# ossamaAhmed/blackbox_mpc

Hardware: AMD Instinct MI355X
Metric: MPC control-steps/sec (agent-control-steps; Pendulum true model, CEM N=500 H=30) (higher is better)
Workload: dtype f32; 1 GPU; BASELINE cfg2: Pendulum-v0 true dynamics, CEM, num_agents=1/GPU, N=500, H=30, 5 iters, k=50, closed loop (the model is the environment); parallelism=single GPU

## Files before the change

### blackbox_mpc_amd/csrc/bbmpc.hip

```cpp
#include "engine.hpp"
#include "abi_util.hpp"
#include "engine_util.hpp"
#include "kernels_corr.hpp"
#include "kernels_elite_carry.hpp"

#include <math.h>
#include <stdio.h>
#include <stdlib.h>
#include <atomic>
#include <functional>
#include <chrono>
#include <mutex>
#include <set>
#include <thread>
#include <utility>

namespace bbmpc {

static std::mutex g_engines_mu;
static std::set<Engine*> g_engines;
static std::atomic<int> g_resident_handles{0};
void note_resident_handle() { g_resident_handles.fetch_add(1, std::memory_order_relaxed); }

void stop_foreign_residents(Engine* self) {
// ... 107 lines not shown
        const bool per_agent = (c.quirks & BBMPC_CMAES_PER_AGENT) != 0;
        const long nn = per_agent ? (long)H * U : (long)A * H * U;
        REQUIRE(nn <= 4096, BBMPC_E_UNSUPPORTED,
                "CMA-ES joint dimension num_agents*H*U > 4096: use BBMPC_CMAES_PER_AGENT (the reference's own "
                "[N,n,n] map_fn stack cannot run at this size either, cma_es.py:13)");
        REQUIRE(per_agent || c.num_agents_global <= c.num_agents, BBMPC_E_UNSUPPORTED,
                "coupled CMA-ES sums rewards over ALL agents and does not shard; use BBMPC_CMAES_PER_AGENT");
        REQUIRE(k <= 1024, BBMPC_E_UNSUPPORTED, "num_elite > 1024 not supported");
    }

    if (c.population_global != 0 || c.population_offset != 0) {
        REQUIRE(c.population_global >= N && c.population_offset >= 0 && c.population_offset + N <= c.population_global, BBMPC_E_INVALID,
                "population_offset / population_global: this handle's particles must lie inside the global population");
        if (c.population_global > N) {
            REQUIRE(c.optimizer != BBMPC_OPT_NONE, BBMPC_E_UNSUPPORTED, "population sharding needs an optimizer (evaluate-only handles roll out what they are given)");
            if (c.optimizer == BBMPC_OPT_CMAES)
                REQUIRE(k <= N && k <= 1024, BBMPC_E_UNSUPPORTED, "sharded CMA-ES: num_elite must not exceed this rank's share of the population (nor 1024)");
        }
    }
    int ndev = 0;
    if (hipGetDeviceCount(&ndev) != hipSuccess || ndev <= 0)
        throw HipError(BBMPC_E_NO_DEVICE, "no HIP device available: this library has no CPU fallback");
    if (c.device >= 0) {
        REQUIRE(c.device < ndev, BBMPC_E_NO_DEVICE, "bbmpc_config.device out of range");
        HIP_CHECK(hipSetDevice(c.device));
    }
    HIP_CHECK(hipGetDevice(&device));
    HIP_CHECK(hipDeviceGetAttribute(&cu_count, hipDeviceAttributeMultiprocessorCount, device));
    {
        int least = 0, greatest = 0;
        HIP_CHECK(hipDeviceGetStreamPriorityRange(&least, &greatest));
        if (!(own_stream = masked_stream_from_env("BBMPC_STREAM_CUS", cu_count)))
            HIP_CHECK(hipStreamCreateWithPriority(&own_stream, hipStreamNonBlocking, greatest));
    }
    stream = own_stream;
    init_tnq_table();

    if (const char* fm = getenv("BBMPC_FUSED")) fused_mode = atoi(fm);
    {
        auto flag = [](const char* n) { return getenv(n) != nullptr; };
        auto ival = [](const char* n, int dflt) { const char* v = getenv(n); return v ? atoi(v) : dflt; };
        sw.cma_svd_v1 = flag("BBMPC_CMA_SVD_V1"); sw.cma_svd_rounds = flag("BBMPC_CMA_SVD_ROUNDS");
        sw.cma_svd_general = flag("BBMPC_CMA_SVD_GENERAL");
        sw.cma_svd_gram = flag("BBMPC_CMA_SVD_GRAM");
        sw.cma_coop = flag("BBMPC_CMA_COOP"); sw.cma_nb = ival("BBMPC_CMA_NB", 0);
        sw.cma_eigh = ival("BBMPC_CMA_EIGH", 1); sw.cma_eigh_fail = flag("BBMPC_CMA_EIGH_FAIL");
        sw.cma_fused = flag("BBMPC_CMA_FUSED");
        sw.mlp_generic = flag("BBMPC_MLP_GENERIC");
        { const int b = ival("BBMPC_MLP_BF16", 0); sw.mlp_bf16 = (b == 1 || b == 3) ? b : 0; }
        sw.mlp_pair = ival("BBMPC_MLP_PAIR", -1); sw.mlp_q4 = ival("BBMPC_MLP_Q4", -1); sw.mlp_q4s = ival("BBMPC_MLP_Q4S", ival("BBMPC_MLP_Q4R", 1)); sw.mlp_w4 = ival("BBMPC_MLP_W4", 1); sw.pi2_skip_init = ival("BBMPC_PI2_SKIP_INIT", 1); sw.step_graph = ival("BBMPC_STEP_GRAPH", 1); sw.cma_small3 = ival("BBMPC_CMA_SMALL3", 1);
        sw.refit_wgs = ival("BBMPC_REFIT_WGS", 0);
        sw.mlp_wave = ival("BBMPC_MLP_WAVE", 1);
        sw.linger_us = std::max(0, ival("BBMPC_LINGER_US", 200));
        linger_test_quit = ival("BBMPC_LINGER_TEST_QUIT", 0) - 1;
        host_seq = (uint32_t)ival("BBMPC_TEST_HOST_SEQ", 0);
        sw.balance = ival("BBMPC_BALANCE", 0);
        sw.ilp = ival("BBMPC_ILP", 1) == 2 ? 2 : 1;
        sw.refit_v1 = flag("BBMPC_REFIT_V1");
        sw.zero_copy = !flag("BBMPC_NO_ZERO_COPY");
        sw.host_poll = !flag("BBMPC_NO_HOST_POLL");
        sw.mlp_no_half_tail = flag("BBMPC_MLP_NO_HALF_TAIL");
        sw.dbg = flag("BBMPC_DBG");
        sw.prof_reward_mlp = flag("BBMPC_PROF_REWARD_MLP");
        user_stepwise_only = flag("BBMPC_USER_STEPWISE");
        if (c.optimizer != BBMPC_OPT_NONE) {
            ps_loopback = auto_split > 1 ? auto_split : ival("BBMPC_POPSHARD_LOOPBACK", 0);
            ps_force = flag("BBMPC_POPSHARD_FORCE");
        }
    }
    HU = H * U;
    Nst = ((std::max(N, 1) + 63) / 64) * 64;
    rec = U + S + 1;
    lo.assign(c.action_low, c.action_low + U);
    hi.assign(c.action_high, c.action_high + U);
    upload(d_lo, lo);
    upload(d_hi, hi);
    d_state.alloc((size_t)A * S);
    d_record.alloc((size_t)A * rec);
    d_action.alloc((size_t)A * U);
    d_action.zero(stream);
    if (c.optimizer != BBMPC_OPT_NONE) {
        std::vector<float> m((size_t)A * HU), v((size_t)A * HU);
        for (int i = 0; i < A * HU; ++i) {
            const int u = i % U;
            m[i] = (lo[u] + hi[u]) / 2.0f;
            const float d = lo[u] - hi[u];
            v[i] = (d * d) / 16.0f;
        }
        upload(d_prev_mean, m);
        upload(d_var0, v);
        d_mean.alloc(m.size());
        d_var.alloc(m.size());
        d_sigma.alloc(m.size());
        d_samples.alloc((size_t)A * HU * Nst);
        d_rewards.alloc((size_t)A * Nst);
        d_penalty.alloc((size_t)A * Nst);
        d_elites.alloc((size_t)A * std::max(k, 1));
        const size_t big = (size_t)A * HU * Nst;
        if (c.optimizer == BBMPC_OPT_SPSA) {
            d_cand_a.alloc(big);
            d_cand_b.alloc(big);
            d_rewards2.alloc((size_t)A * Nst);
        }
        if (c.optimizer == BBMPC_OPT_CMAES) {
            d_cand_a.alloc(big);
            cma_init();
// ... 2145 lines not shown
```

### blackbox_mpc_amd/csrc/bbmpc_fused.hip

```cpp
#define BBMPC_TU_FUSED
#include "engine.hpp"
#include "engine_util.hpp"

#include <atomic>
#include <chrono>

namespace bbmpc {

void bbmpc_tu_fused_upload_tnq(const float2* table) { tnq_upload(table); }

bool Engine::use_fused() const {
    if (cfg.dynamics != BBMPC_DYN_PENDULUM || cfg.reward != BBMPC_REW_PENDULUM) return false;
    if (pop_sharded()) return false;
    if (particles_on()) return false;
    if (corr_on()) return false;
    if (carry_on()) return false;
    if (prior_on()) return false;
    if (grad_on()) return false;
    if (cfg.optimizer == BBMPC_OPT_SPSA) {
        if (iters > FUSED_MAX_SPSA_ITERS) return false;
    } else if (cfg.optimizer != BBMPC_OPT_RANDOM_SEARCH && cfg.optimizer != BBMPC_OPT_CEM && cfg.optimizer != BBMPC_OPT_PI2) {
        return false;
    }
    if (fused_mode == 0) return false;
    if (fused_mode == 1) return true;
    return (long)N <= 2048 || A >= 64;
}

static void note_inst(Engine& e, int opt, bool samples_lds, bool fastm, int inj, int ilp, bool linger) {
    snprintf(e.dominant_inst, sizeof(e.dominant_inst), "k_fused_pendulum<%d, %s, %s, %d, %d, %s>", opt, samples_lds ? "true" : "false",
             fastm ? "true" : "false", inj, ilp, linger ? "true" : "false");
}

template <int OPT, bool FASTM, int INJ, int ILP>
static void launch_fused4(Engine& e, FusedArgs& fa, int threads, size_t lds_base, size_t lds_samples) {
#ifdef BBMPC_KERNEL_DBG
    const size_t limit = 158 * 1024;
#else
    const size_t limit = 160 * 1024;
#endif
    if (lds_base + lds_samples <= limit) {
        fa.test_quit_agent = -1;
        if constexpr (INJ == 2 && FASTM && ILP == 1) {
            if (e.linger_launch && e.subset_n == 0 && fa.done_flag && e.tail.event == nullptr) {
                auto fl = k_fused_pendulum<OPT, true, FASTM, INJ, ILP, true>;
                note_inst(e, OPT, true, FASTM, INJ, ILP, true);
                ensure_max_lds((const void*)fl, (int)limit);
                if (e.rec != kCompletionRecordFloats) throw HipError(BBMPC_E_HIP, "internal: the resident pendulum kernel's record is not 5 floats");
                for (int a = 0; a < e.A; ++a) {
                    volatile uint32_t* m = e.mbox_host(a);
                    volatile uint32_t* cl = e.ack_host(a);
                    for (int i = 0; i < 16; ++i) cl[i] = (fa.done_value - 1u) & 0xffffu;                    for (int i = 0; i < 13; ++i) m[i] = fa.done_value & 0xffffu;
                    m[15] = fa.done_value;
                    *(volatile uint32_t*)e.gone_host(a) = 0u;
                }
                std::atomic_thread_fence(std::memory_order_release);
                fa.done_flag = e.sync_dev(e.ack_host(0));
                fa.mbox = e.sync_dev(e.mbox_host(0));
                fa.gone = e.sync_dev(e.gone_host(0));
                fa.linger_ticks = (unsigned)e.sw.linger_us * 100u;
                fa.test_quit_agent = e.linger_test_quit;
                hipLaunchKernelGGL(fl, dim3(e.A), dim3(threads), lds_base + lds_samples, e.stream, fa);
                HIP_CHECK(hipGetLastError());
                e.resident_alive = true;
                if (!e.mbox_pub.load(std::memory_order_relaxed)) {
                    e.mbox_pub_agents = e.A;
                    e.mbox_pub.store(e.mbox_host(0), std::memory_order_release);
                    note_resident_handle();
                }
                return;
            }
        }
        if (e.subset_n > 0) {
            auto fs = k_fused_pendulum<OPT, true, FASTM, INJ, ILP>;
            note_inst(e, OPT, true, FASTM, INJ, ILP, false);
            ensure_max_lds((const void*)fs, (int)limit);
            fa.amap = reinterpret_cast<const int*>(e.sync_dev(e.amap_host()));
            hipLaunchKernelGGL(fs, dim3(e.subset_n), dim3(threads), lds_base + lds_samples, e.stream, fa);
            HIP_CHECK(hipGetLastError());
            e.subset_n = 0;
            return;
        }
        auto fn = k_fused_pendulum<OPT, true, FASTM, INJ, ILP>;
        note_inst(e, OPT, true, FASTM, INJ, ILP, false);
        ensure_max_lds((const void*)fn, (int)limit);
        launch_with_tail(e, fn, dim3(e.A), dim3(threads), lds_base + lds_samples, fa);
    } else {
        auto fn = k_fused_pendulum<OPT, false, FASTM, INJ, ILP>;
        note_inst(e, OPT, false, FASTM, INJ, ILP, false);
        launch_with_tail(e, fn, dim3(e.A), dim3(threads), lds_base, fa);
    }
    HIP_CHECK(hipGetLastError());
}

template <int OPT>
static void launch_fused(Engine& e, FusedArgs& fa, int ilp, int threads, size_t lds_base, size_t lds_samples, int inj_layout) {
    const bool fastm = !e.fix(BBMPC_STRICT_MATH);
    const int inj = fa.inj == nullptr ? 0 : inj_layout;
#define LF(F, I)                                                                              \
    do {                                                                                      \
        if (ilp == 2) launch_fused4<OPT, F, I, 2>(e, fa, threads, lds_base, lds_samples);    \
        else launch_fused4<OPT, F, I, 1>(e, fa, threads, lds_base, lds_samples);             \
    } while (0)
    if (inj == 2) {
        if (fastm) launch_fused4<OPT, true, 2, 1>(e, fa, threads, lds_base, lds_samples);
        else launch_fused4<OPT, false, 2, 1>(e, fa, threads, lds_base, lds_samples);
    } else if (fastm && !inj) LF(true, 0);
    else if (fastm && inj) LF(true, 1);
    else if (!fastm && !inj) LF(false, 0);
    else LF(false, 1);
#undef LF
}

__global__ void k_noise_fill(RngKey key, uint32_t rstream, int kind , int n_it, int N, int Nst, int A, int Q,
                             int agent_offset, float4* __restrict__ out) {
    const int idx = blockIdx.x * blockDim.x + threadIdx.x;
    if (idx >= N * Q) return;
    const int n = idx / Q, q = idx % Q;
    const int z = blockIdx.y;
    const int a = z % A, it = (z / A) % n_it, s = z / (A * n_it);
    key.step += (uint32_t)s;
    const U4 w = rng_block(key, rstream, (uint32_t)it, (uint32_t)n, (uint32_t)(agent_offset + a), (uint32_t)(4 * q));
    float4 v;
    if (kind == 1) v = make_float4(word_to_uniform(w.x), word_to_uniform(w.y), word_to_uniform(w.z), word_to_uniform(w.w));
    else if (kind == 2) v = make_float4(word_to_rademacher(w.x), word_to_rademacher(w.y), word_to_rademacher(w.z), word_to_rademacher(w.w));
    else v = make_float4(word_to_trunc_normal(w.x), word_to_trunc_normal(w.y), word_to_trunc_normal(w.z), word_to_trunc_normal(w.w));
    out[(((size_t)s * n_it + it) * A + a) * Nst * Q + (size_t)n * Q + q] = v;
}

void Engine::launch_noise_fill(int64_t chunk, int buf, hipStream_t on) {
    const bool rs = cfg.optimizer == BBMPC_OPT_RANDOM_SEARCH, sp = cfg.optimizer == BBMPC_OPT_SPSA;
    const int n_it = rs ? 1 : iters, Q = (HU + 3) / 4;
    dim3 grid((N * Q + 255) / 256, A * n_it * pf_steps), block(256);
    hipLaunchKernelGGL(k_noise_fill, grid, block, 0, on, key((uint32_t)(chunk * pf_steps)), rs ? 2u : (sp ? 3u : 1u), rs ? 1 : (sp ? 2 : 0), n_it,
                       N, Nst, A, Q, cfg.agent_offset, reinterpret_cast<float4*>(d_noise_pf[buf].p));
    HIP_CHECK(hipGetLastError());
}

void Engine::optimize_fused(const float* d_state_in, int add_noise, float* d_record_out, float* d_next_out, uint32_t step) {
    FusedArgs fa;
    memset(&fa, 0, sizeof(fa));
    fa.N = N; fa.A = A; fa.H = H; fa.U = U; fa.HU = HU; fa.Nst = Nst; fa.k = k; fa.iters = iters;
    fa.agent_offset = cfg.agent_offset;
// ... 26 lines not shown
        ensure_trace();
        fa.t_rewards = t_rewards.p; fa.t_mean = t_mean.p; fa.t_var = t_var.p; fa.t_elites = t_elites.p; fa.t_passes = t_passes.p; fa.t_samples = t_samples.p;
        if (cfg.optimizer == BBMPC_OPT_SPSA) {
            if (!t_rewards2.p) t_rewards2.alloc((size_t)A * Nst * std::max(iters, 1));
            fa.t_rewards2 = t_rewards2.p;
        }
    }
#ifdef BBMPC_KERNEL_DBG
    static long long* dbg_buf = nullptr;
    if (sw.dbg) {
        if (!dbg_buf) {
            HIP_CHECK(hipHostMalloc((void**)&dbg_buf, 64 * 8, hipHostMallocDefault));
            memset(dbg_buf, 0, 64 * 8);
        }
        if (dbg_buf[42]) {
            const long long* d = dbg_buf;
            fprintf(stderr, "[dbg] last resident pass, 10ns units rel. to its start:");
            for (int i = 0; i <= 1 + iters * 4; ++i) fprintf(stderr, " %lld", d[i] - d[0]);
            fprintf(stderr, "\n[dbg] iter0 per-wave rollout end:");
            for (int i = 24; i < 32; ++i) fprintf(stderr, " %lld", d[i] - d[0]);
            fprintf(stderr, "\n[dbg] request accepted %lld  first model step %lld  completion stored %lld\n", d[42] - d[0], d[44] - d[0], d[43] - d[0]);
            const long long sel = d[iters > 0 ? 4 * iters : 0];
            fprintf(stderr, "[dbg] tail rel. to the last selection: tail start %lld  noise applied %lld  model step %lld  record stored %lld  published %lld  last barrier %lld  carry stored %lld\n",
                    d[38] - sel, d[35] - sel, d[36] - sel, d[37] - sel, d[43] - sel, d[1 + iters * 4] - sel, d[34] - sel);
            dbg_buf[42] = 0;
        }
        fa.dbg = dbg_buf;
    }
#endif
    fa.key = key(step);
    const int pf_nit = cfg.optimizer == BBMPC_OPT_RANDOM_SEARCH ? 1 : iters;
    if (pf_mode < 0) {
        const char* ev = getenv("BBMPC_NOISE_PREFETCH");
        pf_step_floats = U == 1 ? noise_step_floats(pf_nit, A, Nst, H) : (size_t)pf_nit * A * Nst * ((HU + 3) / 4) * 4;
        const size_t budget = (size_t)128 << 20;
        pf_steps = pf_step_floats ? (int)std::min<size_t>(8, budget / (pf_step_floats * 4)) : 0;
        pf_mode = ((ev ? atoi(ev) != 0 : true) && pf_steps >= 1 && U == 1) ? 1 : 0;
        if (pf_mode) {
            {
                int least = 0, greatest = 0;
                HIP_CHECK(hipDeviceGetStreamPriorityRange(&least, &greatest));
                HIP_CHECK(hipStreamCreateWithPriority(&pf_stream, hipStreamNonBlocking, greatest));
            }
            HIP_CHECK(hipEventCreateWithFlags(&pf_free, hipEventDisableTiming));
            for (int b = 0; b < 2; ++b) {
                const size_t pad = noise_pad_floats(H);
                d_noise_pf[b].alloc(noise_alloc_floats(pf_steps, pf_nit, A, Nst, H));
                HIP_CHECK(hipMemset(d_noise_pf[b].p + pf_step_floats * pf_steps, 0xff, pad * sizeof(float)));
                HIP_CHECK(hipEventCreateWithFlags(&pf_done[b], hipEventDisableTiming));
            }
        }
    }
    const bool use_pf = pf_mode == 1 && fa.inj == nullptr && pf_nit > 0;
    if (use_pf) {
        const int64_t c = (int64_t)step / pf_steps;
        const int pb = (int)(c & 1), nb = pb ^ 1;
        if (pf_chunk[pb] != c) {
            if (pf_inflight[pb]) HIP_CHECK(hipStreamWaitEvent(stream, pf_done[pb], 0));
            launch_noise_fill(c, pb, stream);
            pf_chunk[pb] = c; pf_waited[pb] = true; pf_inflight[pb] = false;
        } else if (!pf_waited[pb]) {
            HIP_CHECK(hipStreamWaitEvent(stream, pf_done[pb], 0));
            pf_waited[pb] = true; pf_inflight[pb] = false;
        }
        fa.inj = d_noise_pf[pb].p + (size_t)((int64_t)step - c * pf_steps) * pf_step_floats;
        fa.pf_buf[0] = d_noise_pf[0].p; fa.pf_buf[1] = d_noise_pf[1].p;
        fa.pf_step_floats = pf_step_floats; fa.pf_chunk_floats = pf_step_floats * (size_t)pf_steps;
        if (pf_chunk[nb] != c + 1) {
            HIP_CHECK(hipEventRecord(pf_free, stream));
            HIP_CHECK(hipStreamWaitEvent(pf_stream, pf_free, 0));
            launch_noise_fill(c + 1, nb, pf_stream);
            HIP_CHECK(hipEventRecord(pf_done[nb], pf_stream));
            pf_chunk[nb] = c + 1; pf_waited[nb] = false; pf_inflight[nb] = true;
        }
    }
    int ilp = 1;
    ilp = sw.ilp;
    if (use_pf) ilp = 1;
    const int per = (N + ilp - 1) / ilp;
    const int threads = std::min(1024, std::max(((per + 63) / 64) * 64, ((std::max(k, 1) + 63) / 64) * 64));
    const int HUp = (HU + 3) & ~3, kp = (std::max(k, 1) + 3) & ~3;
    static_assert(TOPK_HIST_WORDS % 4 == 0, "every piece of the carve is a multiple of 16 bytes");
    static_assert(TOPK_HIST_WORDS_NARROW % 4 == 0, "every piece of the carve is a multiple of 16 bytes");
    const int hist_words = cfg.optimizer == BBMPC_OPT_CEM ? TOPK_HIST_WORDS : TOPK_HIST_WORDS_NARROW;
    const size_t lds_base = (size_t)(Nst + 3 * HUp + kp + 64 + hist_words + 2 * kp) * 4;
    const size_t lds_samples = (size_t)HU * Nst * 4;
    prof_begin();
    switch (cfg.optimizer) {
        case BBMPC_OPT_RANDOM_SEARCH: launch_fused<FOPT_RS>(*this, fa, ilp, threads, lds_base, lds_samples, use_pf ? 2 : 1); break;
        case BBMPC_OPT_CEM: launch_fused<FOPT_CEM>(*this, fa, ilp, threads, lds_base, lds_samples, use_pf ? 2 : 1); break;
        case BBMPC_OPT_SPSA: {
            const bool fastm = !fix(BBMPC_STRICT_MATH);
            if (use_pf) {
                if (fastm) launch_fused4<FOPT_SPSA, true, 2, 1>(*this, fa, threads, lds_base, lds_samples);
                else launch_fused4<FOPT_SPSA, false, 2, 1>(*this, fa, threads, lds_base, lds_samples);
            } else if (fa.inj) {
                if (fastm) launch_fused4<FOPT_SPSA, true, 1, 1>(*this, fa, threads, lds_base, lds_samples);
                else launch_fused4<FOPT_SPSA, false, 1, 1>(*this, fa, threads, lds_base, lds_samples);
            } else {
                if (fastm) launch_fused4<FOPT_SPSA, true, 0, 1>(*this, fa, threads, lds_base, lds_samples);
                else launch_fused4<FOPT_SPSA, false, 0, 1>(*this, fa, threads, lds_base, lds_samples);
            }
            break;
        }
        default: launch_fused<FOPT_PI2>(*this, fa, ilp, threads, lds_base, lds_samples, use_pf ? 2 : 1); break;
    }
// ... 70 lines not shown
```

### blackbox_mpc_amd/csrc/engine.hpp

```cpp
#pragma once
#include <hip/hip_ext.h>
#include <hip/hip_runtime.h>
#include <stdint.h>
#include <string.h>

#include <algorithm>
#include <atomic>
#include <map>
#include <stdexcept>
#include <string>
#include <vector>

#include "../../include/bbmpc.h"
#include "comm.hpp"
#include "completion_line.hpp"
#include "kernels_cma.hpp"
#include "kernels_eigh.hpp"
#include "kernels_eigh_small.hpp"
#include "kernels_fused.hpp"
#include "kernels_fused_cma.hpp"
#include "kernels_fused_pso.hpp"
#include "kernels_mlp.hpp"
#include "kernels_mlp_xform.hpp"
#include "kernels_mlp_q4s.hpp"
// ... 93 lines not shown
        if (flag) attached = true;
        return {flag, count, value};
    }
};

struct Engine {
    bbmpc_config cfg;
    int N, A, H, U, S, HU, Nst, iters, k;
    int rec;
    std::vector<float> lo, hi;
    hipStream_t own_stream = nullptr, stream = nullptr;
    int cu_count = 0;
    int device = 0;
    uint32_t step_counter = 0;
    hipGraphExec_t step_graph = nullptr;
    uint64_t step_graph_sig = 0;
    uint64_t step_warm_sig = 0;
    int step_graph_warm = 0;
    uint32_t mutations = 0;
    uint32_t* step_words_dev = nullptr;
    uint32_t* step_words = nullptr;
    uint32_t step_mirror[2] = {0, 0};
    void ensure_step_words();
    bool step_capturing = false;
    int64_t calls_graph = 0;
    int64_t graph_capture_failures = 0;
    bool last_step_steady = false;
    void invalidate_step_graph() {
        ++mutations;
        step_graph_warm = 0;
        if (step_graph) { (void)hipGraphExecDestroy(step_graph); step_graph = nullptr; }
    }
    bool trace_on = false, profiling = false;
    int prof_every = 1;
    uint64_t prof_seq = 0;
    bool prof_this = false;
    int fused_mode = -1;
    struct Switches {
        bool cma_svd_v1 = false, cma_svd_rounds = false, cma_svd_general = false, cma_svd_gram = false, cma_fused = false, cma_coop = false;
        bool cma_eigh_fail = false;
        int cma_eigh = 1;
        int cma_nb = 0;
        bool mlp_generic = false;
        int mlp_bf16 = 0;
        int mlp_pair = -1, mlp_q4 = -1;
        int mlp_w4 = 1;
        int mlp_q4s = 1;
        int cma_small3 = 1;
        int step_graph = 1;
        int pi2_skip_init = 1;
        int refit_wgs = 0;
        int mlp_wave = 1;
        int linger_us = 200;
        int balance = 0;
        int ilp = 1;
        bool refit_v1 = false;
        bool zero_copy = true;
        bool mlp_no_half_tail = false;
        bool host_poll = true;
        bool prof_reward_mlp = false;
        bool dbg = false;
    } sw;

    DevBuf<float> d_lo, d_hi, d_state, d_record, d_action;
    DevBuf<float> d_prev_mean, d_var0, d_mean, d_var, d_sigma;
    DevBuf<float> d_samples, d_rewards, d_penalty;
    DevBuf<int> d_elites;
    bool mlp_ready = false;
    MlpDesc mlp;
    int mlp_nw = 1;
    DevBuf<float> d_wpack[MLP_MAX_LAYERS], d_wpack4[MLP_MAX_LAYERS], d_bpack[MLP_MAX_LAYERS], d_wraw[MLP_MAX_LAYERS], d_braw[MLP_MAX_LAYERS], d_wq4[MLP_MAX_LAYERS], d_wq4s0, d_w4pack, d_wbf[MLP_MAX_LAYERS], d_stats;
    DevBuf<float> d_fin_next, d_fin_rew, d_step_act;
    DevBuf<float> d_cand_a, d_cand_b, d_rewards2, d_vel, d_pbest, d_pbest_r, d_gbest, d_gbest_r, d_cond;
    DevBuf<int> d_gidx;
    DevBuf<float> t_rewards2;
    bool pso_seeded = false;
    int cma_G = 0, cma_n = 0;
    CmaConst cma_c;
    DevBuf<float> c_w, c_m, c_sigma, c_C, c_B, c_Dd, c_ps, c_pc, c_BD, c_z, c_Ye, c_xm, c_ym, c_evec, c_eval, c_E;
    DevBuf<int> c_eidx, c_info;
    DevBuf<unsigned> c_sync;
    DevBuf<float> e_d, e_e, e_tau, e_Vt, e_alpha, e_lam, e_Z, e_Z2, e_P, e_Tf;
    DevBuf<unsigned> e_flags;
    bool cma_use_eigh_small() const { return sw.cma_eigh && cma_n >= 2 && cma_n <= ES_N && !sw.cma_svd_v1 && !sw.cma_svd_rounds && !sw.cma_svd_general && !sw.cma_svd_gram; }
    bool cma_use_eigh() const { return sw.cma_eigh && cma_n > 128 && cma_n <= EIGH_MAX_N && (cma_n & 3) == 0 && !sw.cma_svd_v1 && !sw.cma_svd_rounds && !sw.cma_svd_general && !sw.cma_svd_gram; }
    void cma_eigh_launch(const CmaArgs& q);
    hipStream_t eigh_side = nullptr;
    hipEvent_t eigh_ev[2] = {nullptr, nullptr};
    int eigh_side_state = -1;
    DevBuf<float> d_eval_rew, d_step_c;
    DevBuf<float> d_stage;
    int stage_depth = 0;
    std::map<int, DevBuf<float>> inj;
    DevBuf<float> t_rewards, t_mean, t_var, t_samples;
    DevBuf<int> t_elites;
    DevBuf<int> t_passes;
    DevBuf<int> t_cma_stats;
    DevBuf<float> t_cma_B, t_cma_C, t_cma_D;
    float* h_pin = nullptr;
    float* h_pin_dev = nullptr;
    size_t h_pin_n = 0;
    DevBuf<float> d_noise_pf[2];
    RecordComm rc;
    DevBuf<float> d_record_slot[RecordComm::kSlots];
    float* h_record_stage[RecordComm::kSlots] = {nullptr, nullptr};
    bool gather_deferred[RecordComm::kSlots] = {false, false};
// ... 337 lines not shown
```

### blackbox_mpc_amd/csrc/kernels_fused.hpp

```cpp
#pragma once
#include <type_traits>

#include "kernels_opt.hpp"
#include "kernels_refit.hpp"
#include "kernels_rollout.hpp"
#include "noise_extent.hpp"
#include "topk.hpp"

namespace bbmpc {

constexpr int FOPT_RS = 1;
constexpr int FOPT_CEM = 2;
constexpr int FOPT_PI2 = 3;
constexpr int FOPT_SPSA = 4;
constexpr int FUSED_MAX_SPSA_ITERS = 16;

struct FusedArgs {
    int N, A, H, U, HU, Nst, k, iters;
    int agent_offset;
    int fix_q1, fix_q7, add_noise;
    int warm_start;
    unsigned* done_flag;
    unsigned* done_count;
    unsigned done_value;
// ... 8 lines not shown
    float* samples_g;
    const float* inj;
    const float* inj_expl;
    float* record;
    float* next_state;
    float spsa_ak[FUSED_MAX_SPSA_ITERS], spsa_ck[FUSED_MAX_SPSA_ITERS];
    float* t_rewards2;
    float* t_rewards;
    float* t_mean;
    float* t_var;
    int* t_elites;
    float* t_samples;
    long long* dbg;
    RngKey key;
    const unsigned* mbox;
    unsigned* gone;
    unsigned linger_ticks;
    int test_quit_agent;
    const int* amap;
    const float* pf_buf[2];
    unsigned long long pf_step_floats, pf_chunk_floats;
    int* t_passes;
};


#ifdef BBMPC_KERNEL_DBG
#define BB_DBG(slot) do { if (p.dbg && tid == 0 && a == 0) dbg_lds[(slot)] = (long long)wall_clock64(); } while (0)
#else
#define BB_DBG(slot) do {} while (0)
#endif

__device__ __forceinline__ float block_min(float v, float* red, int tid, int nw) {
    v = wave_min(v);
    if ((tid & 63) == 0) red[tid >> 6] = v;
    __syncthreads();
    float r = red[(tid & 63) < nw ? (tid & 63) : 0];
    r = wave_min(r);
    __syncthreads();
    return r;
}
__device__ __forceinline__ float block_sum(float v, float* red, int tid, int nw) {
    v = wave_sum(v);
    if ((tid & 63) == 0) red[tid >> 6] = v;
    __syncthreads();
    float r = ((tid & 63) < nw) ? red[tid & 63] : 0.0f;
    r = wave_sum(r);
    __syncthreads();
    return r;
}

#ifndef BBMPC_FUSED_ACTIONS_AHEAD
#define BBMPC_FUSED_ACTIONS_AHEAD 1
#endif
template <int OPT, bool SAMPLES_LDS, bool FASTM, int INJ, int ILP, bool LINGER = false>
__global__ void k_fused_pendulum(FusedArgs p) {
    extern __shared__ __attribute__((aligned(16))) float smem[];
    const int a = p.amap ? p.amap[blockIdx.x] : (int)blockIdx.x;
    const int tid = threadIdx.x;
    const int nthr = blockDim.x;
    const int nw = nthr >> 6;
    const int HUp = (p.HU + 3) & ~3;
    const int kp = (p.k + 3) & ~3;
    float* rew = smem;
    float* mean = rew + p.Nst;
    float* var = mean + HUp;
    float* sigma = var + HUp;
    int* eidx = (int*)(sigma + HUp);
    float* red = (float*)(eidx + kp);
    uint32_t* hist = (uint32_t*)(red + 64);
    unsigned long long* ekeys = (unsigned long long*)(hist + (OPT == FOPT_CEM ? TOPK_HIST_WORDS : TOPK_HIST_WORDS_NARROW));
    float* samp = SAMPLES_LDS ? (float*)(ekeys + kp) : (p.samples_g + (size_t)a * p.HU * p.Nst);
#ifdef BBMPC_KERNEL_DBG
    __shared__ long long dbg_lds[48];
#endif
    const PendulumModel model{p.fix_q1 != 0};
    const float lo = p.lo[0], hi = p.hi[0];
    RngKey key_s = p.key;
    const float* inj_s = p.inj;
    int add_noise_s = p.add_noise;
    unsigned done_value_s = p.done_value;
    if (tid < 3) red[60 + tid] = p.state[a * 3 + tid];
    const bool keep_init = LINGER && OPT != FOPT_RS && p.HU <= nthr;
    [[maybe_unused]] float m_keep = 0.0f, v_keep = 0.0f, s_keep = 0.0f;
    auto dist_init = [&](bool from_keep) {
        if (from_keep) {
            if (tid < p.HU) {
                mean[tid] = m_keep;
                var[tid] = v_keep;
                sigma[tid] = (OPT == FOPT_CEM && p.warm_start) ? cem_sigma(m_keep, v_keep, lo, hi) : s_keep;
            }
        } else {
            for (int j = tid; j < p.HU; j += nthr) {
                const float m = p.prev_mean[a * p.HU + j];
                const float v = p.var0[a * p.HU + j];
                const float sg = (OPT == FOPT_CEM) ? cem_sigma(m, v, lo, hi) : ((OPT == FOPT_SPSA) ? 0.0f : sqrtf(v));
                mean[j] = m;
                var[j] = v;
                sigma[j] = sg;
                if (keep_init) { m_keep = m; v_keep = v; s_keep = sg; }
            }
        }
    };
    typedef float pfvec4 __attribute__((ext_vector_type(4)));
    typedef const __attribute__((address_space(1))) pfvec4* pfvec4p;
    [[maybe_unused]] pfvec4 pf0 = {0.0f, 0.0f, 0.0f, 0.0f}, pf1 = {0.0f, 0.0f, 0.0f, 0.0f};
    [[maybe_unused]] auto prefetch_first = [&](const float* base, int it_n) {
        if constexpr (INJ == 2) {
            const int Q = (p.HU + 3) >> 2;
            if (tid < p.N) {
                const pfvec4p q = (pfvec4p)(reinterpret_cast<const float4*>(base) + noise_block_index(it_n, p.A, a, p.Nst, tid, Q));
                pf0 = q[0];
                if (OPT != FOPT_SPSA) pf1 = q[1];
            }
        }
    };
    dist_init(false);
    __syncthreads();
    float s0 = red[60], s1 = red[61], s2 = red[62];
    if (p.iters > 0) prefetch_first(inj_s, 0);
    auto noise_term = [&]() {
        FinalArgs fa;
        fa.A = p.A; fa.U = 1; fa.S = 3;
        fa.agent_offset = p.agent_offset;
        fa.fix_q1 = p.fix_q1; fa.fix_q7 = p.fix_q7;
        fa.add_noise = add_noise_s;
        fa.lo = p.lo; fa.hi = p.hi;
        fa.inj = p.inj_expl;
        fa.key = key_s;
        fa.key.q_per_agent = 1;
        return exploration_noise(fa, a, 0, lo, hi);
    };
    const bool tail_lanes = LINGER ? tid < 64 : tid == 0;
    auto tail = [&](float act_in) {
        BB_DBG(38);
        float s[3] = {s0, s1, s2};
        float act[1];
        act[0] = add_noise_s ? exploration_apply(act_in, noise_term(), lo, hi) : act_in;
        BB_DBG(35);
        const float r = model.step(s, act);
        BB_DBG(36);
        if constexpr (LINGER) {
            const unsigned tag = done_value_s & 0xffffu;
            const float f = tid < 2 ? act[0] : (tid < 4 ? s[0] : (tid < 6 ? s[1] : (tid < 8 ? s[2] : r)));
            const unsigned bits = __float_as_uint(f);
            unsigned w = ((tid & 1) ? (bits & 0xffff0000u) : (bits << 16)) | tag;
            if (tid >= 10) w = tag;
            if (tid == 15) w = done_value_s;
            if (tid < 16) __hip_atomic_store(p.done_flag + a * 16 + tid, w, __ATOMIC_RELAXED, __HIP_MEMORY_SCOPE_SYSTEM);
            BB_DBG(37);
        } else {
            float* rec = p.record + (size_t)a * 5;
            rec[0] = act[0];
            rec[1] = s[0];
            rec[2] = s[1];
            rec[3] = s[2];
            rec[4] = r;
            if (p.next_state) {
                p.next_state[a * 3 + 0] = s[0];
                p.next_state[a * 3 + 1] = s[1];
                p.next_state[a * 3 + 2] = s[2];
            }
            BB_DBG(37);
            publish_records_done(p.done_flag, p.done_count, done_value_s, gridDim.x);
        }
        BB_DBG(43);
    };
    for (;;) {

        float action0 = (OPT == FOPT_RS) ? 0.0f : mean[0];

        BB_DBG(0);
#ifdef BBMPC_KERNEL_DBG
        if (p.dbg && tid == 0 && a == 0) dbg_lds[40] = (long long)clock64();
#endif
        for (int it = 0; it < p.iters; ++it) {
            BB_DBG(1 + it * 4);
            const float* inj = (INJ == 1) ? inj_s + ((size_t)it * p.A + a) * p.HU * p.Nst : nullptr;
            const int nblk = p.H >> 2, rem = p.H & 3;
            const uint32_t rstream = (OPT == FOPT_RS) ? 2u : 1u;
            auto with_q1 = [&](auto&& body) {
                if constexpr (FASTM) {
                    if (p.fix_q1 != 0) { body(std::true_type{}); return; }
                }
                body(std::false_type{});
            };
            if constexpr (OPT == FOPT_SPSA) {
                const float ck = p.spsa_ck[it];
                const int nb4 = (p.H + 3) >> 2;
                with_q1([&](auto Q1c) {
                constexpr bool Q1 = decltype(Q1c)::value;
                for (int n = tid; n < p.N; n += nthr) {
                    Roller<FASTM> rp, rm;
                    rp.init(p.fix_q1 != 0, s0, s1, s2);
                    rm.init(p.fix_q1 != 0, s0, s1, s2);
                    float tp = 0.0f, tm = 0.0f, pp = 0.0f, pm = 0.0f;
                    typedef float gvec4s __attribute__((ext_vector_type(4)));
                    typedef const __attribute__((address_space(1))) gvec4s* gvec4sp;
                    [[maybe_unused]] gvec4sp mine4 = nullptr;
                    [[maybe_unused]] gvec4s cur4 = {1.0f, 1.0f, 1.0f, 1.0f};
                    if constexpr (INJ == 2) {
                        mine4 = (gvec4sp)(reinterpret_cast<const float4*>(inj_s) + noise_block_index(it, p.A, a, p.Nst, n, nb4));
                        if (n == tid) cur4 = pf0;
                        else cur4 = mine4[0];
                    }
                    for (int b = 0; b < nb4; ++b) {
                        float d[4];
                        if constexpr (INJ == 2) {
                            const gvec4s nxt4 = mine4[b + 1];
                            d[0] = cur4.x; d[1] = cur4.y; d[2] = cur4.z; d[3] = cur4.w;
                            cur4 = nxt4;
                        } else if (INJ == 1) {
#pragma unroll
                            for (int i = 0; i < 4; ++i) d[i] = (4 * b + i < p.H) ? inj[(size_t)(4 * b + i) * p.Nst + n] : 1.0f;
                        } else {
                            const U4 w = rng_block(key_s, 3u, (uint32_t)it, (uint32_t)n, (uint32_t)(p.agent_offset + a), (uint32_t)(4 * b));
                            d[0] = word_to_rademacher(w.x); d[1] = word_to_rademacher(w.y);
                            d[2] = word_to_rademacher(w.z); d[3] = word_to_rademacher(w.w);
                        }
#pragma unroll
                        for (int i = 0; i < 4; ++i) {
                            const int t = 4 * b + i;
                            if (t < p.H) {
                                const float th = mean[t], stp = ck * d[i];
                                const float xp = th + stp, xm = th - stp;
                                const float xpf = clipf(xp, lo, hi), xmf = clipf(xm, lo, hi);
                                const float dp = xp - xpf, dm = xm - xmf;
                                pp = pp + dp * dp;
                                pm = pm + dm * dm;
                                samp[(size_t)t * p.Nst + n] = d[i];
                                rp.template step_acc_q1<Q1>(xpf);
                                rm.template step_acc_q1<Q1>(xmf);
                            }
                        }
                    }
                    tp = rp.total(); tm = rm.total();
                    if (tp != tp) tp = -1.0e6f;
                    if (tm != tm) tm = -1.0e6f;
                    const float np_ = sqrtf(pp), nm_ = sqrtf(pm);
                    const float r_p = tp - np_ * np_, r_m = tm - nm_ * nm_;
                    if (p.t_rewards) {
                        p.t_rewards[((size_t)it * p.A + a) * p.Nst + n] = r_p;
                        p.t_rewards2[((size_t)it * p.A + a) * p.Nst + n] = r_m;
                    }
                    rew[n] = r_p - r_m;
                }
                });
            } else if constexpr (INJ == 2) {
                const int Q = (p.HU + 3) >> 2;
                const float4* inj4 = reinterpret_cast<const float4*>(inj_s);
                auto rollout = [&](auto Q1c, auto NSTc) {
                constexpr bool Q1 = decltype(Q1c)::value;
                constexpr int NSTC = decltype(NSTc)::value;
                const size_t nst = NSTC ? (size_t)NSTC : (size_t)p.Nst;
                for (int n = tid; n < p.N; n += nthr) {
// ... 146 lines not shown
                }
                for (int i = 0; i < rem; ++i)
#pragma unroll
                    for (int q = 0; q < ILP; ++q) consume(q, 4 * nblk + i, xn[q][i]);
#pragma unroll
                for (int q = 0; q < ILP; ++q) {
                    float tot = roll[q].total();
                    if (tot != tot) tot = -1.0e6f;
                    if (OPT == FOPT_PI2) {
                        const float nr = sqrtf(pen[q]);
                        tot = tot - nr * nr;
                    }
                    if (live[q]) rew[nn[q]] = tot;
                }
            }
            });
#ifdef BBMPC_KERNEL_DBG
            if (p.dbg && a == 0 && it == 0 && (tid & 63) == 0) dbg_lds[24 + (tid >> 6) % 8] = (long long)wall_clock64();
#endif
            if (it + 1 < p.iters) prefetch_first(inj_s, it + 1);
            if (OPT == FOPT_CEM) block_topk_prepass(rew, p.N, p.k, hist, tid, nthr);
            BB_DBG(2 + it * 4);
            __syncthreads();
            BB_DBG(3 + it * 4);
            if (p.t_rewards) {
                if (OPT != FOPT_SPSA)
                    for (int n = tid; n < p.N; n += nthr) p.t_rewards[((size_t)it * p.A + a) * p.Nst + n] = rew[n];
                for (int i = tid; i < p.HU * p.Nst; i += nthr) {
                    const int j = i / p.Nst, n = i % p.Nst;
                    if (n < p.N) p.t_samples[(((size_t)it * p.A + a) * p.HU + j) * p.Nst + n] = samp[(size_t)j * p.Nst + n];
                }
            }

            if (OPT == FOPT_CEM) {
                const TopkSel sel = block_topk_select(rew, p.N, p.k, hist, tid, nthr, true);
                if (p.t_passes && tid == 0) p.t_passes[(size_t)it * p.A + a] = sel.passes;
                if (p.t_elites) {
                    block_topk_finish_sorted(rew, p.N, p.k, eidx, hist, ekeys, sel, tid, nthr);
                    for (int e = tid; e < p.k; e += nthr) p.t_elites[((size_t)it * p.A + a) * p.k + e] = eidx[e];
                    __syncthreads();
                }
                block_topk_finish_indexed(rew, p.N, p.k, eidx, hist, sel, tid, nthr);
                BB_DBG(4 + it * 4);
#ifdef BBMPC_KERNEL_DBG
                if (p.dbg && tid == 0 && a == 0 && it == 1) for (int i = 0; i < 12; ++i) p.dbg[48 + i] = g_topk_dbg[i];
#endif
                const float kf = (float)p.k;
                const int sub = tid & 15;
                constexpr int EC = 4;
                const bool small_k = p.k <= 16 * EC;
                int ei[EC];
#pragma unroll
                for (int i = 0; i < EC; ++i) ei[i] = (small_k && sub + 16 * i < p.k) ? eidx[sub + 16 * i] : -1;
                for (int j = tid >> 4; j < ((p.HU + 3) & ~3); j += nthr >> 4) {
                    const bool live = j < p.HU;
                    const float* row = samp + (size_t)(live ? j : 0) * p.Nst;
                    float sum = 0.0f, vs = 0.0f, em;
                    if (small_k) {
                        float x[EC];
#pragma unroll
                        for (int i = 0; i < EC; ++i) x[i] = row[ei[i] >= 0 ? ei[i] : 0];
#pragma unroll
                        for (int i = 0; i < EC; ++i) if (ei[i] >= 0) sum += x[i];
                        sum = row16_sum(sum);
                        em = sum / kf;
#pragma unroll
                        for (int i = 0; i < EC; ++i)
                            if (ei[i] >= 0) {
                                const float d = x[i] - em;
                                vs += d * d;
                            }
                    } else {
                        for (int e = sub; e < p.k; e += 16) sum += row[eidx[e]];
                        sum = row16_sum(sum);
                        em = sum / kf;
                        for (int e = sub; e < p.k; e += 16) {
                            const float d = row[eidx[e]] - em;
                            vs += d * d;
                        }
                    }
                    vs = row16_sum(vs);
                    if (live && sub == 0) {
                        const float ev = vs / kf;
                        const float one_m = 1.0f - p.alpha;
                        const float m = p.alpha * mean[j] + one_m * em;
                        const float v = p.alpha * var[j] + one_m * ev;
                        mean[j] = m;
                        var[j] = v;
                        sigma[j] = cem_sigma(m, v, lo, hi);
                    }
                }
                if (it == 0) BB_DBG(33);
                __syncthreads();
                action0 = mean[0];
            } else if (OPT == FOPT_PI2) {
                float lmin = INFINITY;
                for (int n = tid; n < p.N; n += nthr) {
                    const float c = -rew[n];
                    rew[n] = c;
                    lmin = fminf(lmin, c);
                }
                lmin = wave_min(lmin);
                if ((tid & 63) == 0) red[tid >> 6] = lmin;
                __syncthreads();
                float beta = ((tid & 63) < nw) ? red[tid & 63] : INFINITY;
                beta = wave_min(beta);
                float lsum = 0.0f;
                for (int n = tid; n < p.N; n += nthr) {
                    const float pr = expf((-p.inv_lamda) * (rew[n] - beta));
                    rew[n] = pr;
                    lsum += pr;
                }
                lsum = wave_sum(lsum);
                if ((tid & 63) == 0) red[32 + (tid >> 6)] = lsum;
                __syncthreads();
                float eta = ((tid & 63) < nw) ? red[32 + (tid & 63)] : 0.0f;
                eta = wave_sum(eta);
                const float inv_eta = 1.0f / eta;
                for (int j = tid >> 6; j < p.HU; j += nw) {
                    const float* row = samp + (size_t)j * p.Nst;
                    float acc = 0.0f;
                    for (int n = tid & 63; n < p.N; n += 64) acc += row[n] * (inv_eta * rew[n]);
                    acc = wave_sum(acc);
                    if ((tid & 63) == 0) mean[j] = acc;
                }
                __syncthreads();
                action0 = mean[0];
            } else if (OPT == FOPT_SPSA) {
                const float two_ck = 2.0f * p.spsa_ck[it], ak = p.spsa_ak[it];
                for (int j = tid >> 6; j < p.HU; j += nw) {
                    const float* row = samp + (size_t)j * p.Nst;
                    float acc = 0.0f;
                    for (int n = tid & 63; n < p.N; n += 64) acc += rew[n] / (two_ck * row[n]);
                    acc = wave_sum(acc);
                    if ((tid & 63) == 0) mean[j] = clipf(mean[j] + ak * (acc / (float)p.N), lo, hi);
                }
                __syncthreads();
                action0 = mean[0];
            } else {
                float bv = -INFINITY;
                int bi = 0x7fffffff;
                for (int n = tid; n < p.N; n += nthr) {
                    const float v = rew[n];
                    if (v > bv || (v == bv && n < bi)) { bv = v; bi = n; }
                }
                wave_argmax(bv, bi);
                int* redi = (int*)(red + 32);
                if ((tid & 63) == 0) { red[tid >> 6] = bv; redi[tid >> 6] = bi; }
                __syncthreads();
                bv = ((tid & 63) < nw) ? red[tid & 63] : -INFINITY;
                bi = ((tid & 63) < nw) ? redi[tid & 63] : 0x7fffffff;
                wave_argmax(bv, bi);
                if (bi == 0x7fffffff) bi = 0;
                action0 = samp[bi];
                if (p.t_elites && tid == 0) p.t_elites[a] = bi;
                __syncthreads();
            }
            if (p.t_mean && OPT != FOPT_RS)
                for (int j = tid; j < p.HU; j += nthr) {
                    p.t_mean[((size_t)it * p.A + a) * p.HU + j] = mean[j];
                    p.t_var[((size_t)it * p.A + a) * p.HU + j] = var[j];
                }
        }

        BB_DBG(1 + p.iters * 4);
#ifdef BBMPC_KERNEL_DBG
        if (p.dbg && tid == 0 && a == 0) dbg_lds[41] = (long long)clock64();
#endif
        if (tail_lanes) tail(action0);
        if (OPT != FOPT_RS) {
            for (int j = tid; j < p.HU; j += nthr) {
                p.mean_out[a * p.HU + j] = mean[j];
                p.var_out[a * p.HU + j] = var[j];
                if (OPT == FOPT_PI2 || OPT == FOPT_SPSA) {
                    const int js = (j + 1 < p.HU) ? j + 1 : p.HU - 1;
                    const float pm = mean[js];
                    p.prev_mean[a * p.HU + j] = pm;
                    if (keep_init) m_keep = pm;
                } else if (p.warm_start) {
                    const float pm = mean[j];
                    p.prev_mean[a * p.HU + j] = pm;
                    if (keep_init) m_keep = pm;
                }
            }
        }
        BB_DBG(34);
#ifdef BBMPC_KERNEL_DBG
        if (p.dbg && a == 0 && tid == 0) for (int i = 0; i < 48; ++i) p.dbg[i] = dbg_lds[i];
#endif
        if constexpr (!LINGER) {
            break;
        } else {
            unsigned* mb = (unsigned*)(red + 16);
            __syncthreads();
            dist_init(keep_init);
            [[maybe_unused]] const float* inj_pred = nullptr;
            if constexpr (INJ == 2) {
                if (p.pf_step_floats)
                    for (int b = 0; b < 2; ++b)
                        if (inj_s >= p.pf_buf[b] && inj_s + 2 * p.pf_step_floats <= p.pf_buf[b] + p.pf_chunk_floats) inj_pred = inj_s + p.pf_step_floats;
                if (inj_pred && p.iters > 0) prefetch_first(inj_pred, 0);
            }
            if (tid < 64) {
                const long long t0 = (long long)wall_clock64();
                const unsigned want = done_value_s + 1u;
                unsigned w = 0u;
                bool quit = false;
                for (;;) {
                    w = (tid < 16) ? __hip_atomic_load(p.mbox + a * 16 + tid, __ATOMIC_RELAXED, __HIP_MEMORY_SCOPE_SYSTEM) : 0u;
                    const bool mine = tid < 13 ? (w & 0xffffu) == (want & 0xffffu) : (tid == 15 ? w == want : true);
                    const unsigned w15 = __builtin_amdgcn_readlane(w, 15);
                    if (__builtin_amdgcn_ballot_w64(mine) == ~0ull) break;
                    if (w15 == 0xffffffffu || (long long)wall_clock64() - t0 > (long long)p.linger_ticks || a == p.test_quit_agent || (p.test_quit_agent >= 999 && a >= p.test_quit_agent - 999)) { quit = true; break; }
                }
                if (tid < 16) mb[tid] = (quit && tid == 15) ? 0xffffffffu : w;
                BB_DBG(42);
            }
            __syncthreads();
            if (mb[15] == 0xffffffffu) {
                if (tid == 0) __hip_atomic_store(p.gone + a * 16, done_value_s, __ATOMIC_RELEASE, __HIP_MEMORY_SCOPE_SYSTEM);
                return;
            }
// ... 15 lines not shown
```

Before: 33000 control-steps/s.

## Add 512-thread launch-bounded fused CEM kernel and run the tail early

Adds a MAXT template parameter with __launch_bounds__ so the fused pendulum CEM kernel can be compiled for at most 512 threads when the launch fits, giving the compiler a larger register budget. In that form the closed-loop tail (environment step and completion record) runs right after the last CEM refit, on the lanes that computed mean row 0, instead of after the final barrier and output writes. This moves the tail off the end of the step's critical path. The cost is more template instantiations and a more complex ordering for the tail lanes, and EARLY_TAIL assumes those lanes hold mean_row0.

Measured after the change: 34360 control-steps/s (median of 6 runs). +4.1%, better.

```diff
diff --git a/blackbox_mpc_amd/csrc/bbmpc.hip b/blackbox_mpc_amd/csrc/bbmpc.hip
--- a/blackbox_mpc_amd/csrc/bbmpc.hip
+++ b/blackbox_mpc_amd/csrc/bbmpc.hip
@@ -183,6 +183,10 @@
         sw.refit_wgs = ival("BBMPC_REFIT_WGS", 0);
         sw.mlp_wave = ival("BBMPC_MLP_WAVE", 1);
         sw.linger_us = std::max(0, ival("BBMPC_LINGER_US", 200));
+        if (const char* fb = getenv("BBMPC_FUSED_BOUND")) {
+            sw.fused_bound = atoi(fb);
+            REQUIRE(sw.fused_bound == 512 || sw.fused_bound == 1024, BBMPC_E_INVALID, "BBMPC_FUSED_BOUND must be 512, 1024 or unset");
+        }
         linger_test_quit = ival("BBMPC_LINGER_TEST_QUIT", 0) - 1;
         host_seq = (uint32_t)ival("BBMPC_TEST_HOST_SEQ", 0);
         sw.balance = ival("BBMPC_BALANCE", 0);
diff --git a/blackbox_mpc_amd/csrc/bbmpc_fused.hip b/blackbox_mpc_amd/csrc/bbmpc_fused.hip
--- a/blackbox_mpc_amd/csrc/bbmpc_fused.hip
+++ b/blackbox_mpc_amd/csrc/bbmpc_fused.hip
@@ -27,24 +27,47 @@
     return (long)N <= 2048 || A >= 64;
 }
 
-static void note_inst(Engine& e, int opt, bool samples_lds, bool fastm, int inj, int ilp, bool linger) {
-    snprintf(e.dominant_inst, sizeof(e.dominant_inst), "k_fused_pendulum<%d, %s, %s, %d, %d, %s>", opt, samples_lds ? "true" : "false",
-             fastm ? "true" : "false", inj, ilp, linger ? "true" : "false");
-}
+static constexpr size_t fused_lds_limit() {
+#ifdef BBMPC_KERNEL_DBG
+    return 158 * 1024;
+#else
+    return 160 * 1024;
+#endif
+}
+
+static void note_inst(Engine& e, int opt, bool samples_lds, bool fastm, int inj, int ilp, int maxt, bool linger) {
+    snprintf(e.dominant_inst, sizeof(e.dominant_inst), "k_fused_pendulum<%d, %s, %s, %d, %d, %d, %s>", opt, samples_lds ? "true" : "false",
+             fastm ? "true" : "false", inj, ilp, maxt, linger ? "true" : "false");
+}
+
+template <int OPT, int INJ, int ILP>
+constexpr bool fused_has_bound512() { return OPT == FOPT_CEM && (INJ == 2 || INJ == 1) && ILP == 1; }
+
+template <int OPT, bool FASTM, int INJ, int ILP, int MAXT>
+static void launch_fused5(Engine& e, FusedArgs& fa, int threads, size_t lds_base, size_t lds_samples);
 
 template <int OPT, bool FASTM, int INJ, int ILP>
 static void launch_fused4(Engine& e, FusedArgs& fa, int threads, size_t lds_base, size_t lds_samples) {
-#ifdef BBMPC_KERNEL_DBG
-    const size_t limit = 158 * 1024;
-#else
-    const size_t limit = 160 * 1024;
-#endif
+    if constexpr (fused_has_bound512<OPT, INJ, ILP>()) {
+        if (threads <= 512 && e.sw.fused_bound != 1024 && lds_base + lds_samples <= fused_lds_limit()) {
+            REQUIRE(threads <= 512, BBMPC_E_HIP, "internal: a 512-bounded k_fused_pendulum launched with more threads");
+            launch_fused5<OPT, FASTM, INJ, ILP, 512>(e, fa, threads, lds_base, lds_samples);
+            return;
+        }
+    }
+    REQUIRE(threads <= 1024, BBMPC_E_HIP, "internal: k_fused_pendulum launched with more than 1024 threads");
+    launch_fused5<OPT, FASTM, INJ, ILP, 1024>(e, fa, threads, lds_base, lds_samples);
+}
+
+template <int OPT, bool FASTM, int INJ, int ILP, int MAXT>
+static void launch_fused5(Engine& e, FusedArgs& fa, int threads, size_t lds_base, size_t lds_samples) {
+    const size_t limit = fused_lds_limit();
     if (lds_base + lds_samples <= limit) {
         fa.test_quit_agent = -1;
         if constexpr (INJ == 2 && FASTM && ILP == 1) {
             if (e.linger_launch && e.subset_n == 0 && fa.done_flag && e.tail.event == nullptr) {
-                auto fl = k_fused_pendulum<OPT, true, FASTM, INJ, ILP, true>;
-                note_inst(e, OPT, true, FASTM, INJ, ILP, true);
+                auto fl = k_fused_pendulum<OPT, true, FASTM, INJ, ILP, MAXT, true>;
+                note_inst(e, OPT, true, FASTM, INJ, ILP, MAXT, true);
                 ensure_max_lds((const void*)fl, (int)limit);
                 if (e.rec != kCompletionRecordFloats) throw HipError(BBMPC_E_HIP, "internal: the resident pendulum kernel's record is not 5 floats");
                 for (int a = 0; a < e.A; ++a) {
@@ -72,8 +95,8 @@
             }
         }
         if (e.subset_n > 0) {
-            auto fs = k_fused_pendulum<OPT, true, FASTM, INJ, ILP>;
-            note_inst(e, OPT, true, FASTM, INJ, ILP, false);
+            auto fs = k_fused_pendulum<OPT, true, FASTM, INJ, ILP, MAXT>;
+            note_inst(e, OPT, true, FASTM, INJ, ILP, MAXT, false);
             ensure_max_lds((const void*)fs, (int)limit);
             fa.amap = reinterpret_cast<const int*>(e.sync_dev(e.amap_host()));
             hipLaunchKernelGGL(fs, dim3(e.subset_n), dim3(threads), lds_base + lds_samples, e.stream, fa);
@@ -81,14 +104,16 @@
             e.subset_n = 0;
             return;
         }
-        auto fn = k_fused_pendulum<OPT, true, FASTM, INJ, ILP>;
-        note_inst(e, OPT, true, FASTM, INJ, ILP, false);
+        auto fn = k_fused_pendulum<OPT, true, FASTM, INJ, ILP, MAXT>;
+        note_inst(e, OPT, true, FASTM, INJ, ILP, MAXT, false);
         ensure_max_lds((const void*)fn, (int)limit);
         launch_with_tail(e, fn, dim3(e.A), dim3(threads), lds_base + lds_samples, fa);
+    } else if constexpr (MAXT == 1024) {
+        auto fn = k_fused_pendulum<OPT, false, FASTM, INJ, ILP>;
+        note_inst(e, OPT, false, FASTM, INJ, ILP, 1024, false);
+        launch_with_tail(e, fn, dim3(e.A), dim3(threads), lds_base, fa);
     } else {
-        auto fn = k_fused_pendulum<OPT, false, FASTM, INJ, ILP>;
-        note_inst(e, OPT, false, FASTM, INJ, ILP, false);
-        launch_with_tail(e, fn, dim3(e.A), dim3(threads), lds_base, fa);
+        throw HipError(BBMPC_E_HIP, "internal: the samples-in-global k_fused_pendulum has no 512-thread form");
     }
     HIP_CHECK(hipGetLastError());
 }
@@ -221,6 +246,7 @@
         }
     }
     const bool use_pf = pf_mode == 1 && fa.inj == nullptr && pf_nit > 0;
+    REQUIRE(!use_pf || U == 1, BBMPC_E_HIP, "internal: prefetched draws need U == 1");
     if (use_pf) {
         const int64_t c = (int64_t)step / pf_steps;
         const int pb = (int)(c & 1), nb = pb ^ 1;
diff --git a/blackbox_mpc_amd/csrc/engine.hpp b/blackbox_mpc_amd/csrc/engine.hpp
--- a/blackbox_mpc_amd/csrc/engine.hpp
+++ b/blackbox_mpc_amd/csrc/engine.hpp
@@ -169,6 +169,7 @@
         int refit_wgs = 0;
         int mlp_wave = 1;
         int linger_us = 200;
+        int fused_bound = 0;
         int balance = 0;
         int ilp = 1;
         bool refit_v1 = false;
diff --git a/blackbox_mpc_amd/csrc/kernels_fused.hpp b/blackbox_mpc_amd/csrc/kernels_fused.hpp
--- a/blackbox_mpc_amd/csrc/kernels_fused.hpp
+++ b/blackbox_mpc_amd/csrc/kernels_fused.hpp
@@ -84,8 +84,12 @@
 #ifndef BBMPC_FUSED_ACTIONS_AHEAD
 #define BBMPC_FUSED_ACTIONS_AHEAD 1
 #endif
-template <int OPT, bool SAMPLES_LDS, bool FASTM, int INJ, int ILP, bool LINGER = false>
-__global__ void k_fused_pendulum(FusedArgs p) {
+#ifndef BBMPC_FUSED_EARLY_TAIL
+#define BBMPC_FUSED_EARLY_TAIL 1
+#endif
+template <int OPT, bool SAMPLES_LDS, bool FASTM, int INJ, int ILP, int MAXT = 1024, bool LINGER = false>
+__global__ __launch_bounds__(MAXT) void k_fused_pendulum(FusedArgs p) {
+    static_assert(MAXT == 512 || MAXT == 1024, "k_fused_pendulum: a launch bound of 512 or 1024 threads");
     extern __shared__ __attribute__((aligned(16))) float smem[];
     const int a = p.amap ? p.amap[blockIdx.x] : (int)blockIdx.x;
     const int tid = threadIdx.x;
@@ -162,10 +166,12 @@
         fa.key.q_per_agent = 1;
         return exploration_noise(fa, a, 0, lo, hi);
     };
+    constexpr bool EARLY_TAIL = BBMPC_FUSED_EARLY_TAIL && MAXT == 512 && OPT == FOPT_CEM;
     const bool tail_lanes = LINGER ? tid < 64 : tid == 0;
     auto tail = [&](float act_in) {
         BB_DBG(38);
         float s[3] = {s0, s1, s2};
+        if constexpr (EARLY_TAIL) asm volatile("" : "+v"(s[0]), "+v"(s[1]), "+v"(s[2]));
         float act[1];
         act[0] = add_noise_s ? exploration_apply(act_in, noise_term(), lo, hi) : act_in;
         BB_DBG(35);
@@ -231,7 +237,7 @@
                     [[maybe_unused]] gvec4sp mine4 = nullptr;
                     [[maybe_unused]] gvec4s cur4 = {1.0f, 1.0f, 1.0f, 1.0f};
                     if constexpr (INJ == 2) {
-                        mine4 = (gvec4sp)(reinterpret_cast<const float4*>(inj_s) + noise_block_index(it, p.A, a, p.Nst, n, nb4));
+                        mine4 = (gvec4sp)(reinterpret_cast<const float4*>(inj_s) + noise_block_index(it, p.A, a, p.Nst, n, (p.HU + 3) >> 2));
                         if (n == tid) cur4 = pf0;
                         else cur4 = mine4[0];
                     }
@@ -484,6 +490,7 @@
                 int ei[EC];
 #pragma unroll
                 for (int i = 0; i < EC; ++i) ei[i] = (small_k && sub + 16 * i < p.k) ? eidx[sub + 16 * i] : -1;
+                [[maybe_unused]] float mean_row0 = 0.0f;
                 for (int j = tid >> 4; j < ((p.HU + 3) & ~3); j += nthr >> 4) {
                     const bool live = j < p.HU;
                     const float* row = samp + (size_t)(live ? j : 0) * p.Nst;
@@ -520,9 +527,15 @@
                         mean[j] = m;
                         var[j] = v;
                         sigma[j] = cem_sigma(m, v, lo, hi);
+                        if constexpr (EARLY_TAIL) { if (j == 0) mean_row0 = m; }
                     }
                 }
                 if (it == 0) BB_DBG(33);
+                if constexpr (EARLY_TAIL) {
+                    if (it + 1 == p.iters && tail_lanes) {
+                        tail(__int_as_float(__builtin_amdgcn_readfirstlane(__float_as_int(mean_row0))));
+                    }
+                }
                 __syncthreads();
                 action0 = mean[0];
             } else if (OPT == FOPT_PI2) {
@@ -599,7 +612,7 @@
 #ifdef BBMPC_KERNEL_DBG
         if (p.dbg && tid == 0 && a == 0) dbg_lds[41] = (long long)clock64();
 #endif
-        if (tail_lanes) tail(action0);
+        if (tail_lanes && !(EARLY_TAIL && p.iters > 0)) tail(action0);
         if (OPT != FOPT_RS) {
             for (int j = tid; j < p.HU; j += nthr) {
                 p.mean_out[a * p.HU + j] = mean[j];
```
